# lavajuno/afskmodem

Hardware: AMD Instinct MI355X
Metric: Msamples/s demodulated (batched 48 kHz streams) + decoded-byte match rate vs CPU ref (higher is better)
Workload: dtype int16

## Files before the change

afskmodem_amd/csrc/afsk_synth.hip:

```cpp
#include "afsk_kernels.h"

#include <type_traits>

namespace afsk {

typedef uint32_t store16 __attribute__((ext_vector_type(4), aligned(2)));


__device__ __forceinline__ uint32_t hamming_codeword(uint32_t nib) {
    const uint32_t d1 = (nib >> 3) & 1u, d2 = (nib >> 2) & 1u, d3 = (nib >> 1) & 1u, d4 = nib & 1u;
    return (d1 ^ d2 ^ d4) | ((d1 ^ d3 ^ d4) << 1) | (d1 << 2) | ((d2 ^ d3 ^ d4) << 3) | (d2 << 4) |
           (d3 << 5) | (d4 << 6);
}

constexpr int kModThreads = 256;
constexpr int kModIters = 8;
constexpr int mod_chunk(int iters, int threads = kModThreads) { return threads * 8 * iters; }
constexpr int kWinBytes = 512;

__device__ __forceinline__ bool symbol_is_mark(uint32_t S, uint32_t n_train_sym, uint32_t first_byte,
                                               const uint8_t* win) {
    const uint32_t t = S - n_train_sym;
    const uint32_t b = t - 4u;
    const uint32_t cw = b / 7u;
    const uint32_t pos = b - cw * 7u;
    const uint32_t byte = win[((cw >> 1) - first_byte) & (kWinBytes - 1)];
    const uint32_t nib = (cw & 1u) ? (byte & 15u) : (byte >> 4);
    const bool data_bit = ((hamming_codeword(nib) >> pos) & 1u) != 0;
    const bool train = S < n_train_sym;
    const bool term = t < 4u;
    return train ? ((S & 1u) == 0) : (term ? (t == 0u) : data_bit);
}

constexpr int q_words(int chunk) { return chunk / 32 + 16; }

constexpr uint32_t kHi2 = 0x7FFF7FFFu, kLo2 = 0x80008000u;

template <bool QUIRK, bool SMALLQ>
__device__ __forceinline__ store16 tone_words(uint32_t x0, uint32_t q, float rcp_q, uint32_t mq,
                                              const uint32_t* qb) {
    const uint32_t Q0 = (uint32_t)(((float)x0 + 0.5f) * rcp_q);
    const uint32_t r0 = x0 - Q0 * q;
    const uint32_t bits = __builtin_amdgcn_alignbit(qb[(Q0 >> 5) + 1u], qb[Q0 >> 5], Q0 & 31u);
    store16 w;
    if constexpr (!SMALLQ) {
        const uint32_t c = q - r0;
        if constexpr (QUIRK) {
            const uint32_t d0 = (bits & 1u) ? kHi2 : kLo2, d1 = (bits & 2u) ? kHi2 : kLo2;
#pragma unroll
            for (uint32_t d = 0; d < 4; d++) w[d] = 2u * d < c ? d0 : d1;
        } else {
            const uint32_t l0 = (bits & 1u) ? 0x7FFFu : 0x8000u, l1 = (bits & 2u) ? 0x7FFFu : 0x8000u;
            const uint32_t h0 = l0 << 16, h1 = l1 << 16;
#pragma unroll
            for (uint32_t d = 0; d < 4; d++) w[d] = (2u * d < c ? l0 : l1) | (2u * d + 1u < c ? h0 : h1);
        }
    } else {
        auto hi = [&](uint32_t j) -> bool {
            const uint32_t dq = ((r0 + j) * mq) >> 16;
            return (bits >> dq) & 1u;
        };
#pragma unroll
        for (uint32_t d = 0; d < 4; d++) {
            if constexpr (QUIRK) w[d] = hi(2u * d) ? kHi2 : kLo2;
            else w[d] = (hi(2u * d) ? 0x7FFFu : 0x8000u) | (hi(2u * d + 1u) ? 0x7FFF0000u : 0x80000000u);
        }
    }
    return w;
}

template <int ITERS, int THREADS, bool QUIRK, bool SMALLQ, bool TAIL>
__device__ __forceinline__ void tone_block(int16_t* dst0, uint32_t base, uint32_t len, uint32_t phb,
                                           uint32_t q, const uint32_t* qb, uint32_t lim) {
    const float rcp_q = 1.0f / (float)q;
    const uint32_t mq = (65536u + q - 1u) / q;
#pragma unroll
    for (int it = 0; it < ITERS; it++) {
        const uint32_t local = ((uint32_t)it * THREADS + threadIdx.x) * 8u;
        const uint32_t p0 = base + local;
        if (p0 >= len) break;
        store16 w = tone_words<QUIRK, SMALLQ>(phb + local, q, rcp_q, mq, qb);
        if constexpr (TAIL) {
#pragma unroll
            for (uint32_t d = 0; d < 4; d++) w[d] = p0 + 2u * d < lim ? w[d] : 0u;
        }
        int16_t* dst = dst0 + p0;
        if (p0 + 8u <= len) {
            *reinterpret_cast<store16*>(dst) = w;
        } else {
#pragma unroll
            for (uint32_t j = 0; j < 8u; j++)
                if (p0 + j < len) dst[j] = (int16_t)(w[j >> 1] >> (16u * (j & 1u)));
        }
    }
}

template <int ITERS, int THREADS = kModThreads>
__global__ __launch_bounds__(THREADS) void modulate_kernel_t(ModulateArgs a) {
    constexpr int kModChunk = mod_chunk(ITERS, THREADS);
    static_assert(kModChunk / 56 + 4 <= kWinBytes, "payload window too small for the block");
    __shared__ uint8_t win[kWinBytes];
    __shared__ unsigned long long kinds[kModChunk / 4 / 64 + 2];
    __shared__ uint32_t qbits[q_words(kModChunk)];
    const int bid = xcd_block((int)blockIdx.x, (int)gridDim.x);
    const int s = bid / a.chunks;
    const int chunk = bid - s * a.chunks;
    if ((uint32_t)a.stream_len[s] > (uint32_t)a.max_len) return;
    const uint32_t len = (uint32_t)a.stream_len[s];
    const uint32_t base = (uint32_t)chunk * kModChunk;
    if (base >= len) return;
    const uint32_t bf = (uint32_t)a.bit_frames[s];
    const uint32_t plen = (uint32_t)a.payload_len[s];
    const uint32_t n_train_sym = 2u * (uint32_t)a.ts_cycles[s];
    const uint32_t n_sym = n_train_sym + 4u + 14u * plen;
    const uint8_t* payload = a.payload + (int64_t)s * a.payload_stride;
    const uint64_t n_tones64 = (uint64_t)n_sym * bf;
    const uint64_t n_frames64 = n_tones64 + 4800u;
    const uint64_t n_out64 = a.wav_quirk ? (n_frames64 & ~1ull) : n_frames64;
    const uint32_t n_tones = n_tones64 > 0xFFFFFFFFull ? 0xFFFFFFFFu : (uint32_t)n_tones64;
    const uint32_t n_out = n_out64 > 0xFFFFFFFFull ? 0xFFFFFFFFu : (uint32_t)n_out64;
    const bool bf_ok = bf >= 4u && bf <= (1u << 20) && (bf & 3u) == 0u;
    const uint32_t lim = bf_ok ? (n_tones < n_out ? n_tones : n_out) : 0u;
    int16_t* dst0 = a.samples + a.stream_offset[s];

    if (base >= lim) {
#pragma unroll
        for (int it = 0; it < ITERS; it++) {
            const uint32_t p0 = base + ((uint32_t)it * THREADS + threadIdx.x) * 8u;
            if (p0 >= len) break;
            int16_t* dst = dst0 + p0;
            if (p0 + 8u <= len) {
                *reinterpret_cast<store16*>(dst) = store16{0u, 0u, 0u, 0u};
            } else {
                for (uint32_t j = 0; j < 8u; j++)
                    if (p0 + j < len) dst[j] = 0;
            }
        }
        return;
    }

    const uint32_t data0 = n_train_sym + 4u;
    const uint32_t Sb = base / bf;
    const uint32_t first_byte = ((Sb > data0 ? Sb - data0 : 0u) / 7u) >> 1;
    const uint32_t last = (base + kModChunk - 1u) / bf + 2u;
    const uint32_t nsym_blk = last - Sb + 1u;
    if (Sb + nsym_blk > data0) {
        for (uint32_t k = threadIdx.x; k < (uint32_t)kWinBytes; k += THREADS) {
            const uint32_t idx = first_byte + k;
            win[k] = idx < plen ? payload[idx] : (uint8_t)0;
        }
        __syncthreads();
    }
    {
        const uint32_t lane = threadIdx.x & 63u, wave = threadIdx.x >> 6;
        for (uint32_t r0 = wave * 64u; r0 < nsym_blk; r0 += THREADS) {
            const uint32_t S = Sb + r0 + lane;
            const bool mk = S < n_sym && symbol_is_mark(S, n_train_sym, first_byte, win);
            const unsigned long long m = __ballot(mk);
            if (lane == 0) kinds[r0 >> 6] = m;
        }
    }
    __syncthreads();
    const uint32_t phb = base - Sb * bf;

    {
        const uint32_t nwords = (nsym_blk + 7u) >> 3;
        for (uint32_t w = threadIdx.x; w <= nwords; w += THREADS) {
            uint32_t x = w < nwords ? (uint32_t)(kinds[w >> 3] >> ((w & 7u) * 8u)) & 0xFFu : 0u;
            x = (x | (x << 12)) & 0x000F000Fu;
            x = (x | (x << 6)) & 0x03030303u;
            x = (x | (x << 3)) & 0x11111111u;
            qbits[w] = 0x33333333u ^ (x * 6u);
        }
        __syncthreads();
        const uint32_t q = bf >> 2;
        const bool tail = base + kModChunk + 8u > lim;
        auto run = [&](auto quirk, auto smallq) {
            if (tail) tone_block<ITERS, THREADS, decltype(quirk)::value, decltype(smallq)::value, true>(dst0, base, len, phb, q, qbits, lim);
            else tone_block<ITERS, THREADS, decltype(quirk)::value, decltype(smallq)::value, false>(dst0, base, len, phb, q, qbits, lim);
        };
        if (a.wav_quirk) {
            if (q >= 8u) run(std::true_type{}, std::false_type{});
            else run(std::true_type{}, std::true_type{});
        } else {
            if (q >= 8u) run(std::false_type{}, std::false_type{});
            else run(std::false_type{}, std::true_type{});
        }
    }
}

__device__ __forceinline__ uint32_t hash32(uint32_t x) {
    x ^= x >> 16; x *= 0x7feb352dU; x ^= x >> 15; x *= 0x846ca68bU; x ^= x >> 16;
    return x;
}

__global__ __launch_bounds__(256) void noise_kernel(NoiseArgs a) {
    const int s = blockIdx.x / a.chunks;
    const int chunk = blockIdx.x - s * a.chunks;
    const int32_t len = a.stream_len[s];
    if ((uint32_t)len > (uint32_t)a.max_len) return;
    const int64_t p0 = ((int64_t)chunk * blockDim.x + threadIdx.x) * 8;
    if (p0 >= len) return;
    const int64_t scale = a.scale_q24[s];
    const uint32_t key = hash32(a.seed ^ hash32(a.stream_idx_base + (uint32_t)s + 0x9e3779b9U));
    int16_t* dst = a.samples + a.stream_offset[s] + p0;
    for (int j = 0; j < 8 && p0 + j < len; j++) {
        const uint32_t t = (uint32_t)(p0 + j);
        int32_t sum = 0;
#pragma unroll
        for (uint32_t k = 0; k < 8; k++) {
            const uint32_t hsh = hash32(key ^ (t * 8u + k));
            sum += (int32_t)(hsh & 0xffffu) + (int32_t)(hsh >> 16);
        }
        const int64_t centred = (int64_t)sum - 524280;
        const int64_t noise = (centred * scale + (1 << 23)) >> 24;
        int64_t v = (int64_t)dst[j] + noise;
        v = v > 32767 ? 32767 : (v < -32768 ? -32768 : v);
        dst[j] = (int16_t)v;
    }
}

template <int ITERS, int THREADS = kModThreads>
hipError_t launch_modulate_t(ModulateArgs a, int32_t max_len, hipStream_t stream) {
    if (a.n_streams <= 0 || max_len <= 0) return hipSuccess;
    const int per_block = mod_chunk(ITERS, THREADS);
    a.chunks = (max_len + per_block - 1) / per_block;
    a.max_len = max_len;
    const int64_t blocks = (int64_t)a.chunks * a.n_streams;
    if (blocks > 0x7fffffffll) return hipErrorInvalidValue;
    hipLaunchKernelGGL((modulate_kernel_t<ITERS, THREADS>), dim3((uint32_t)blocks), dim3(THREADS), 0, stream, a);
    return hipGetLastError();
}

hipError_t launch_modulate(ModulateArgs a, int32_t max_len, hipStream_t stream) {
    return launch_modulate_t<kModIters>(a, max_len, stream);
}

hipError_t launch_noise(NoiseArgs a, int32_t max_len, hipStream_t stream) {
    if (a.n_streams <= 0 || max_len <= 0) return hipSuccess;
    const int per_block = 256 * 8;
    a.chunks = (max_len + per_block - 1) / per_block;
    a.max_len = max_len;
    const int64_t blocks = (int64_t)a.chunks * a.n_streams;
    if (blocks > 0x7fffffffll) return hipErrorInvalidValue;
    hipLaunchKernelGGL(noise_kernel, dim3((uint32_t)blocks), dim3(256), 0, stream, a);
    return hipGetLastError();
}

}

#include "afsk_live_tx.hip"
```

Baseline: 3.785 million.

## Make modulate kernel wave-independent with register symbol masks, no shared memory

Reworks the modulate kernel so each wave handles its own small span of samples. A wave builds its symbol mark/space mask in registers by ballot and reads payload bytes directly from global memory, replacing the shared-memory payload window, kinds and qbits arrays and their block-wide barriers. Per-wave work shrinks from 8 stores per thread to 1, which means more blocks and repeated payload reads across waves. Division by the bit-frame count now uses a uniform magic-reciprocal routine.

```diff
diff --git a/afskmodem_amd/csrc/afsk_synth.hip b/afskmodem_amd/csrc/afsk_synth.hip
--- a/afskmodem_amd/csrc/afsk_synth.hip
+++ b/afskmodem_amd/csrc/afsk_synth.hip
@@ -13,18 +13,20 @@
            (d3 << 5) | (d4 << 6);
 }
 
-constexpr int kModThreads = 256;
-constexpr int kModIters = 8;
-constexpr int mod_chunk(int iters, int threads = kModThreads) { return threads * 8 * iters; }
+constexpr int kModWaves = 4;
+constexpr int kModStores = 1;
+constexpr int mod_span(int stores) { return 64 * 8 * stores; }
 constexpr int kWinBytes = 512;
 
-__device__ __forceinline__ bool symbol_is_mark(uint32_t S, uint32_t n_train_sym, uint32_t first_byte,
-                                               const uint8_t* win) {
+__device__ __forceinline__ uint32_t symbol_byte_index(uint32_t S, uint32_t n_train_sym) {
+    return ((S - n_train_sym - 4u) / 7u) >> 1;
+}
+
+__device__ __forceinline__ bool symbol_kind(uint32_t S, uint32_t n_train_sym, uint32_t byte) {
     const uint32_t t = S - n_train_sym;
     const uint32_t b = t - 4u;
     const uint32_t cw = b / 7u;
     const uint32_t pos = b - cw * 7u;
-    const uint32_t byte = win[((cw >> 1) - first_byte) & (kWinBytes - 1)];
     const uint32_t nib = (cw & 1u) ? (byte & 15u) : (byte >> 4);
     const bool data_bit = ((hamming_codeword(nib) >> pos) & 1u) != 0;
     const bool train = S < n_train_sym;
@@ -32,9 +34,43 @@
     return train ? ((S & 1u) == 0) : (term ? (t == 0u) : data_bit);
 }
 
+__device__ __forceinline__ bool symbol_is_mark(uint32_t S, uint32_t n_train_sym, uint32_t first_byte,
+                                               const uint8_t* win) {
+    return symbol_kind(S, n_train_sym, win[(symbol_byte_index(S, n_train_sym) - first_byte) & (kWinBytes - 1)]);
+}
+
 constexpr int q_words(int chunk) { return chunk / 32 + 16; }
 
 constexpr uint32_t kHi2 = 0x7FFF7FFFu, kLo2 = 0x80008000u;
+
+template <bool QUIRK, bool SMALLQ>
+__device__ __forceinline__ store16 quarter_words(uint32_t r0, uint32_t q, uint32_t mq, uint32_t bits) {
+    store16 w;
+    if constexpr (!SMALLQ) {
+        const uint32_t c = q - r0;
+        if constexpr (QUIRK) {
+            const uint32_t d0 = (bits & 1u) ? kHi2 : kLo2, d1 = (bits & 2u) ? kHi2 : kLo2;
+#pragma unroll
+            for (uint32_t d = 0; d < 4; d++) w[d] = 2u * d < c ? d0 : d1;
+        } else {
+            const uint32_t l0 = (bits & 1u) ? 0x7FFFu : 0x8000u, l1 = (bits & 2u) ? 0x7FFFu : 0x8000u;
+            const uint32_t h0 = l0 << 16, h1 = l1 << 16;
+#pragma unroll
+            for (uint32_t d = 0; d < 4; d++) w[d] = (2u * d < c ? l0 : l1) | (2u * d + 1u < c ? h0 : h1);
+        }
+    } else {
+        auto hi = [&](uint32_t j) -> bool {
+            const uint32_t dq = ((r0 + j) * mq) >> 16;
+            return (bits >> dq) & 1u;
+        };
+#pragma unroll
+        for (uint32_t d = 0; d < 4; d++) {
+            if constexpr (QUIRK) w[d] = hi(2u * d) ? kHi2 : kLo2;
+            else w[d] = (hi(2u * d) ? 0x7FFFu : 0x8000u) | (hi(2u * d + 1u) ? 0x7FFF0000u : 0x80000000u);
+        }
+    }
+    return w;
+}
 
 template <bool QUIRK, bool SMALLQ>
 __device__ __forceinline__ store16 tone_words(uint32_t x0, uint32_t q, float rcp_q, uint32_t mq,
@@ -42,44 +78,71 @@
     const uint32_t Q0 = (uint32_t)(((float)x0 + 0.5f) * rcp_q);
     const uint32_t r0 = x0 - Q0 * q;
     const uint32_t bits = __builtin_amdgcn_alignbit(qb[(Q0 >> 5) + 1u], qb[Q0 >> 5], Q0 & 31u);
-    store16 w;
-    if constexpr (!SMALLQ) {
-        const uint32_t c = q - r0;
-        if constexpr (QUIRK) {
-            const uint32_t d0 = (bits & 1u) ? kHi2 : kLo2, d1 = (bits & 2u) ? kHi2 : kLo2;
-#pragma unroll
-            for (uint32_t d = 0; d < 4; d++) w[d] = 2u * d < c ? d0 : d1;
-        } else {
-            const uint32_t l0 = (bits & 1u) ? 0x7FFFu : 0x8000u, l1 = (bits & 2u) ? 0x7FFFu : 0x8000u;
-            const uint32_t h0 = l0 << 16, h1 = l1 << 16;
-#pragma unroll
-            for (uint32_t d = 0; d < 4; d++) w[d] = (2u * d < c ? l0 : l1) | (2u * d + 1u < c ? h0 : h1);
-        }
-    } else {
-        auto hi = [&](uint32_t j) -> bool {
-            const uint32_t dq = ((r0 + j) * mq) >> 16;
-            return (bits >> dq) & 1u;
-        };
-#pragma unroll
-        for (uint32_t d = 0; d < 4; d++) {
-            if constexpr (QUIRK) w[d] = hi(2u * d) ? kHi2 : kLo2;
-            else w[d] = (hi(2u * d) ? 0x7FFFu : 0x8000u) | (hi(2u * d + 1u) ? 0x7FFF0000u : 0x80000000u);
-        }
-    }
-    return w;
-}
-
-template <int ITERS, int THREADS, bool QUIRK, bool SMALLQ, bool TAIL>
-__device__ __forceinline__ void tone_block(int16_t* dst0, uint32_t base, uint32_t len, uint32_t phb,
-                                           uint32_t q, const uint32_t* qb, uint32_t lim) {
-    const float rcp_q = 1.0f / (float)q;
-    const uint32_t mq = (65536u + q - 1u) / q;
-#pragma unroll
-    for (int it = 0; it < ITERS; it++) {
-        const uint32_t local = ((uint32_t)it * THREADS + threadIdx.x) * 8u;
+    return quarter_words<QUIRK, SMALLQ>(r0, q, mq, bits);
+}
+
+__device__ __forceinline__ uint32_t uniform_div_magic(uint32_t d) {
+    const float r = __builtin_amdgcn_rcpf((float)d) * 4294965248.0f;
+    uint32_t z;
+    asm("v_readfirstlane_b32 %0, %1" : "=s"(z) : "v"((uint32_t)r));
+    return z + __umulhi(z, (0u - d) * z);
+}
+__device__ __forceinline__ uint32_t uniform_div(uint32_t n, uint32_t d, uint32_t z) {
+    uint32_t qt = __umulhi(n, z);
+    uint32_t r = n - qt * d;
+    if (r >= d) { qt++; r -= d; }
+    if (r >= d) qt++;
+    return qt;
+}
+
+template <int STORES>
+struct WaveKinds {
+    static constexpr int kMasks = (mod_span(STORES) / 4 + 63) / 64;
+    static constexpr int kWords = 2 * kMasks + 1;
+    uint32_t w[kWords];
+};
+
+template <int STORES, bool QUIRK, bool SMALLQ, bool TAIL, bool WIDE>
+__device__ __forceinline__ void tone_wave(int16_t* dst0, uint32_t base, uint32_t len, uint32_t ph, uint32_t q,
+                                          uint32_t zbf, const WaveKinds<STORES>& kinds, uint32_t lim) {
+    const float rcp_q = __builtin_amdgcn_rcpf((float)q);
+    const uint32_t mq = SMALLQ ? uniform_div(4u * 65535u + 4u * q, 4u * q, zbf) : 0u;
+    const uint32_t lane = threadIdx.x & 63u;
+    const unsigned long long m0 = ((unsigned long long)kinds.w[1] << 32) | kinds.w[0];
+#pragma unroll
+    for (int it = 0; it < STORES; it++) {
+        const uint32_t local = ((uint32_t)it * 64u + lane) * 8u;
         const uint32_t p0 = base + local;
         if (p0 >= len) break;
-        store16 w = tone_words<QUIRK, SMALLQ>(phb + local, q, rcp_q, mq, qb);
+        const uint32_t x0 = ph + local;
+        const uint32_t Q0 = (uint32_t)(((float)x0 + 0.5f) * rcp_q);
+        const uint32_t r0 = x0 - __umul24(Q0, q);
+        const uint32_t s0 = Q0 >> 2;
+        uint32_t k;
+        if constexpr (WIDE) {
+            const uint32_t i = s0 >> 5;
+            uint32_t lo = 0u, hi = 0u;
+#pragma unroll
+            for (uint32_t j = 0; j + 1u < (uint32_t)WaveKinds<STORES>::kWords; j++) {
+                lo = i == j ? kinds.w[j] : lo;
+                hi = i == j ? kinds.w[j + 1u] : hi;
+            }
+            k = __builtin_amdgcn_alignbit(hi, lo, s0 & 31u);
+        } else {
+            k = (uint32_t)(m0 >> (s0 & 63u));
+        }
+        uint32_t x;
+        if constexpr (SMALLQ) {
+            x = k & 0xFFu;
+            x = (x | (x << 12)) & 0x000F000Fu;
+            x = (x | (x << 6)) & 0x03030303u;
+            x = (x | (x << 3)) & 0x11111111u;
+        } else {
+            x = k & 3u;
+            x = (x | (x << 3)) & 0x11u;
+        }
+        const uint32_t bits = (0x33333333u ^ (x * 6u)) >> (Q0 & 3u);
+        store16 w = quarter_words<QUIRK, SMALLQ>(r0, q, mq, bits);
         if constexpr (TAIL) {
 #pragma unroll
             for (uint32_t d = 0; d < 4; d++) w[d] = p0 + 2u * d < lim ? w[d] : 0u;
@@ -95,19 +158,18 @@
     }
 }
 
-template <int ITERS, int THREADS = kModThreads>
-__global__ __launch_bounds__(THREADS) void modulate_kernel_t(ModulateArgs a) {
-    constexpr int kModChunk = mod_chunk(ITERS, THREADS);
-    static_assert(kModChunk / 56 + 4 <= kWinBytes, "payload window too small for the block");
-    __shared__ uint8_t win[kWinBytes];
-    __shared__ unsigned long long kinds[kModChunk / 4 / 64 + 2];
-    __shared__ uint32_t qbits[q_words(kModChunk)];
+template <int STORES, int WAVES = kModWaves>
+__global__ __launch_bounds__(64 * WAVES) void modulate_kernel_t(ModulateArgs a) {
+    constexpr uint32_t kSpan = (uint32_t)mod_span(STORES);
+    using Kinds = WaveKinds<STORES>;
     const int bid = xcd_block((int)blockIdx.x, (int)gridDim.x);
     const int s = bid / a.chunks;
     const int chunk = bid - s * a.chunks;
+    const uint32_t wave = (uint32_t)__builtin_amdgcn_readfirstlane((int)(threadIdx.x >> 6));
+    const uint32_t lane = threadIdx.x & 63u;
     if ((uint32_t)a.stream_len[s] > (uint32_t)a.max_len) return;
     const uint32_t len = (uint32_t)a.stream_len[s];
-    const uint32_t base = (uint32_t)chunk * kModChunk;
+    const uint32_t base = ((uint32_t)chunk * WAVES + wave) * kSpan;
     if (base >= len) return;
     const uint32_t bf = (uint32_t)a.bit_frames[s];
     const uint32_t plen = (uint32_t)a.payload_len[s];
@@ -125,8 +187,8 @@
 
     if (base >= lim) {
 #pragma unroll
-        for (int it = 0; it < ITERS; it++) {
-            const uint32_t p0 = base + ((uint32_t)it * THREADS + threadIdx.x) * 8u;
+        for (int it = 0; it < STORES; it++) {
+            const uint32_t p0 = base + ((uint32_t)it * 64u + lane) * 8u;
             if (p0 >= len) break;
             int16_t* dst = dst0 + p0;
             if (p0 + 8u <= len) {
@@ -139,53 +201,54 @@
         return;
     }
 
-    const uint32_t data0 = n_train_sym + 4u;
-    const uint32_t Sb = base / bf;
-    const uint32_t first_byte = ((Sb > data0 ? Sb - data0 : 0u) / 7u) >> 1;
-    const uint32_t last = (base + kModChunk - 1u) / bf + 2u;
-    const uint32_t nsym_blk = last - Sb + 1u;
-    if (Sb + nsym_blk > data0) {
-        for (uint32_t k = threadIdx.x; k < (uint32_t)kWinBytes; k += THREADS) {
-            const uint32_t idx = first_byte + k;
-            win[k] = idx < plen ? payload[idx] : (uint8_t)0;
-        }
-        __syncthreads();
-    }
-    {
-        const uint32_t lane = threadIdx.x & 63u, wave = threadIdx.x >> 6;
-        for (uint32_t r0 = wave * 64u; r0 < nsym_blk; r0 += THREADS) {
-            const uint32_t S = Sb + r0 + lane;
-            const bool mk = S < n_sym && symbol_is_mark(S, n_train_sym, first_byte, win);
-            const unsigned long long m = __ballot(mk);
-            if (lane == 0) kinds[r0 >> 6] = m;
-        }
-    }
-    __syncthreads();
-    const uint32_t phb = base - Sb * bf;
-
-    {
-        const uint32_t nwords = (nsym_blk + 7u) >> 3;
-        for (uint32_t w = threadIdx.x; w <= nwords; w += THREADS) {
-            uint32_t x = w < nwords ? (uint32_t)(kinds[w >> 3] >> ((w & 7u) * 8u)) & 0xFFu : 0u;
-            x = (x | (x << 12)) & 0x000F000Fu;
-            x = (x | (x << 6)) & 0x03030303u;
-            x = (x | (x << 3)) & 0x11111111u;
-            qbits[w] = 0x33333333u ^ (x * 6u);
-        }
-        __syncthreads();
-        const uint32_t q = bf >> 2;
-        const bool tail = base + kModChunk + 8u > lim;
-        auto run = [&](auto quirk, auto smallq) {
-            if (tail) tone_block<ITERS, THREADS, decltype(quirk)::value, decltype(smallq)::value, true>(dst0, base, len, phb, q, qbits, lim);
-            else tone_block<ITERS, THREADS, decltype(quirk)::value, decltype(smallq)::value, false>(dst0, base, len, phb, q, qbits, lim);
-        };
-        if (a.wav_quirk) {
-            if (q >= 8u) run(std::true_type{}, std::false_type{});
-            else run(std::true_type{}, std::true_type{});
-        } else {
-            if (q >= 8u) run(std::false_type{}, std::false_type{});
-            else run(std::false_type{}, std::true_type{});
-        }
+    const uint32_t end = base + kSpan < lim ? base + kSpan : lim;
+    const uint32_t zbf = uniform_div_magic(bf);
+    const uint32_t Sb = uniform_div(base, bf, zbf), Se = uniform_div(end - 1u, bf, zbf);
+    const uint32_t ph = base - Sb * bf;
+    const uint32_t nsym = Se - Sb + 1u;
+    Kinds kinds;
+    if (Se < n_train_sym) {
+        const uint32_t pat = (Sb & 1u) ? 0xAAAAAAAAu : 0x55555555u;
+#pragma unroll
+        for (int j = 0; j < Kinds::kWords; j++) kinds.w[j] = pat;
+    } else {
+        const uint32_t data0 = n_train_sym + 4u;
+#pragma unroll
+        for (int p = 0; p < Kinds::kMasks; p++) {
+            unsigned long long m = 0ull;
+            if ((uint32_t)p * 64u < nsym) {
+                const uint32_t S = Sb + (uint32_t)p * 64u + lane;
+                const uint32_t idx = symbol_byte_index(S, n_train_sym);
+                const uint32_t byte = (S >= data0 && idx < plen) ? (uint32_t)payload[idx] : 0u;
+                m = __ballot((S < n_sym) & symbol_kind(S, n_train_sym, byte));
+            }
+            kinds.w[2 * p] = (uint32_t)m;
+            kinds.w[2 * p + 1] = (uint32_t)(m >> 32);
+        }
+        kinds.w[Kinds::kWords - 1] = 0u;
+    }
+
+    const uint32_t q = bf >> 2;
+    const bool tail = base + kSpan + 8u > lim;
+    const bool wide = nsym > 64u;
+    auto run = [&](auto quirk, auto smallq) {
+        constexpr bool Q = decltype(quirk)::value, SQ = decltype(smallq)::value;
+        if constexpr (SQ || mod_span(STORES) / 32 + 1 > 64) {
+            if (wide) {
+                if (tail) tone_wave<STORES, Q, SQ, true, true>(dst0, base, len, ph, q, zbf, kinds, lim);
+                else tone_wave<STORES, Q, SQ, false, true>(dst0, base, len, ph, q, zbf, kinds, lim);
+                return;
+            }
+        }
+        if (tail) tone_wave<STORES, Q, SQ, true, false>(dst0, base, len, ph, q, zbf, kinds, lim);
+        else tone_wave<STORES, Q, SQ, false, false>(dst0, base, len, ph, q, zbf, kinds, lim);
+    };
+    if (a.wav_quirk) {
+        if (q >= 8u) run(std::true_type{}, std::false_type{});
+        else run(std::true_type{}, std::true_type{});
+    } else {
+        if (q >= 8u) run(std::false_type{}, std::false_type{});
+        else run(std::false_type{}, std::true_type{});
     }
 }
 
@@ -220,20 +283,20 @@
     }
 }
 
-template <int ITERS, int THREADS = kModThreads>
+template <int STORES, int WAVES = kModWaves>
 hipError_t launch_modulate_t(ModulateArgs a, int32_t max_len, hipStream_t stream) {
     if (a.n_streams <= 0 || max_len <= 0) return hipSuccess;
-    const int per_block = mod_chunk(ITERS, THREADS);
+    const int per_block = mod_span(STORES) * WAVES;
     a.chunks = (max_len + per_block - 1) / per_block;
     a.max_len = max_len;
     const int64_t blocks = (int64_t)a.chunks * a.n_streams;
     if (blocks > 0x7fffffffll) return hipErrorInvalidValue;
-    hipLaunchKernelGGL((modulate_kernel_t<ITERS, THREADS>), dim3((uint32_t)blocks), dim3(THREADS), 0, stream, a);
+    hipLaunchKernelGGL((modulate_kernel_t<STORES, WAVES>), dim3((uint32_t)blocks), dim3(64 * WAVES), 0, stream, a);
     return hipGetLastError();
 }
 
 hipError_t launch_modulate(ModulateArgs a, int32_t max_len, hipStream_t stream) {
-    return launch_modulate_t<kModIters>(a, max_len, stream);
+    return launch_modulate_t<kModStores>(a, max_len, stream);
 }
 
 hipError_t launch_noise(NoiseArgs a, int32_t max_len, hipStream_t stream) {
@@ -249,4 +312,6 @@
 
 }
 
+#ifndef AFSK_SYNTH_KERNELS_ONLY
 #include "afsk_live_tx.hip"
+#endif
```

Result: slower. 3.748 million (-1.0%).
